# chungimungi/GMLM

Measured on AMD Instinct MI355X. Metric: nodes/sec fwd+bwd (full-batch GraphTextLM step), higher is better.
Workload: dtype bf16; 1 GPU; squirrel-size synthetic graph x1 (N=5201, E=217073, F_in=2089), hidden_channels=768, BERT geometry 768x12, 1257 active text nodes, 16..128 tokens, plm_batch_size=4096; global_nodes=5201, parallelism=single GPU, activation_checkpointing=False, plm_gradient_checkpointing=False, world=1, hip_graph=False, gemm_algorithms=library picks from gmlm_amd/tunable/gfx950.csv (TunableOp lookup)

## Files before the change

gmlm_amd/csrc/wgrad_kernels.hip:

```cpp
#include "attn_common.hpp"

namespace gmlm {

namespace wg {
constexpr int BT = 32;
constexpr int TILE = 256;
constexpr int NW = 8;
constexpr int NBUF = 4;
constexpr int IMG = BT * TILE * 2;
constexpr int STAGE = 2 * IMG;
constexpr int LDS = NBUF * STAGE;
constexpr int PIECES = IMG / 1024 / NW;
constexpr int VM_PER_STAGE = 2 * PIECES;
__device__ __forceinline__ int swz(int r) { return 2 * ((r & 3) | (((r >> 3) & 1) << 2)); }
}

struct WgradParams {
  const bf16_t* dy;
  const bf16_t* x;
  float* part;
  int64_t ld_dy, ld_x, n, k;
  int32_t stages, splits, tiles_k, tiles, remap;
};

__device__ __forceinline__ uint32_t wg_src_off(int64_t ld, int w, int lane) {
  const int row = 2 * w + (lane >> 5), slot = lane & 31;
  return 2u * (uint32_t)(row * ld + 8 * (slot ^ wg::swz(row)));
}

__device__ __forceinline__ void wg_dma(const bf16_t* base, uint32_t off, uint32_t lds) {
  const uint32_t dst = __builtin_amdgcn_readfirstlane(lds);
  uint32_t keep;
  asm volatile("s_mov_b32 %0, m0\n\ts_mov_b32 m0, %3\n\ts_nop 0\n\tglobal_load_lds_dwordx4 %1, %2\n\ts_mov_b32 m0, %0"
               : "=&s"(keep) : "v"(off), "s"(base), "s"(dst) : "memory");
}

__global__ __launch_bounds__(wg::NW * 64, 1) void wgrad_bf16_kernel(WgradParams p) {
  using namespace wg;
  extern __shared__ __attribute__((aligned(1024))) unsigned char smem_dyn[];
  const uint32_t lds0 = (uint32_t)(size_t)(__attribute__((address_space(3))) void*)smem_dyn;
  const int tid = threadIdx.x, lane = tid & 63, w = __builtin_amdgcn_readfirstlane(tid >> 6);
  const uint32_t nwg = gridDim.x, id = blockIdx.x;
  uint32_t lid = id;
  if (p.remap) {
    const uint32_t q = nwg >> 3, r = nwg & 7, xcd = id & 7;
    lid = (xcd < r ? xcd * (q + 1) : r * (q + 1) + (xcd - r) * q) + (id >> 3);
  }
  const int slice = (int)(lid / (uint32_t)p.tiles), tile = (int)(lid % (uint32_t)p.tiles);
  const int n0 = (tile / p.tiles_k) * TILE, k0 = (tile % p.tiles_k) * TILE;
  const int st0 = (int)((int64_t)slice * p.stages / p.splits), st1 = (int)((int64_t)(slice + 1) * p.stages / p.splits);
  const int ns = st1 - st0;

  const uint32_t offa = wg_src_off(p.ld_dy, w, lane), offb = wg_src_off(p.ld_x, w, lane);
  const bf16_t* ga = p.dy + (int64_t)st0 * BT * p.ld_dy + n0;
  const bf16_t* gb = p.x + (int64_t)st0 * BT * p.ld_x + k0;
  const int64_t stepa = (int64_t)BT * p.ld_dy, stepb = (int64_t)BT * p.ld_x;
  auto issue = [&](int s) {
    const uint32_t buf = lds0 + (uint32_t)((s % NBUF) * STAGE) + 1024u * (uint32_t)w;
    const bf16_t* a = ga + s * stepa;
    const bf16_t* b = gb + s * stepb;
#pragma unroll
    for (int k = 0; k < PIECES; ++k) {
      wg_dma(a + (int64_t)(16 * k) * p.ld_dy, offa, buf + 1024u * (uint32_t)(NW * k));
      wg_dma(b + (int64_t)(16 * k) * p.ld_x, offb, buf + (uint32_t)IMG + 1024u * (uint32_t)(NW * k));
    }
  };

  const int g = lane >> 4, q = (lane >> 2) & 3, pp = lane & 3;
  const int wr = w >> 2, wc = w & 3;
  const int row = 8 * g + q, sw = swz(row);
  const uint32_t rbase = (uint32_t)(row * (TILE * 2)) + 8u * (uint32_t)(pp & 1);
  uint32_t aoff[8], boff[4];
#pragma unroll
  for (int m = 0; m < 8; ++m) aoff[m] = rbase + 16u * (uint32_t)((((wr * 128 + 16 * m) >> 3) + (pp >> 1)) ^ sw);
#pragma unroll
  for (int j = 0; j < 4; ++j) boff[j] = (uint32_t)IMG + rbase + 16u * (uint32_t)((((wc * 64 + 16 * j) >> 3) + (pp >> 1)) ^ sw);

  typedef __attribute__((ext_vector_type(4))) float f32x4;
  f32x4 acc[8][4];
#pragma unroll
  for (int m = 0; m < 8; ++m)
#pragma unroll
    for (int j = 0; j < 4; ++j) acc[m][j] = f32x4{0.f, 0.f, 0.f, 0.f};

  const int pre = ns < NBUF - 1 ? ns : NBUF - 1;
  for (int s = 0; s < pre; ++s) issue(s);
  int issued = pre;
  for (int s = 0; s < ns; ++s) {
    const int younger = issued - s - 1;
    if (younger >= 2) asm volatile("s_waitcnt vmcnt(8)" ::: "memory");
    else if (younger == 1) asm volatile("s_waitcnt vmcnt(4)" ::: "memory");
    else asm volatile("s_waitcnt vmcnt(0)" ::: "memory");
    static_assert(VM_PER_STAGE == 4 && NBUF == 4, "vmcnt immediates above assume 4 per stage and 2 younger stages");
    __builtin_amdgcn_s_barrier();
    asm volatile("" ::: "memory");
    if (issued < ns) { issue(issued); ++issued; }
    const unsigned char* img = smem_dyn + (s % NBUF) * STAGE;
    bf16x8 a[8], b[4];
#pragma unroll
    for (int j = 0; j < 4; ++j) {
      const bf16x4 lo = __builtin_amdgcn_ds_read_tr16_b64_v4bf16(GMLM_LDS3(bf16x4, img + boff[j]));
      const bf16x4 hi = __builtin_amdgcn_ds_read_tr16_b64_v4bf16(GMLM_LDS3(bf16x4, img + boff[j] + 4 * TILE * 2));
      b[j] = bf16x8{lo[0], lo[1], lo[2], lo[3], hi[0], hi[1], hi[2], hi[3]};
    }
#pragma unroll
    for (int m = 0; m < 8; ++m) {
      const bf16x4 lo = __builtin_amdgcn_ds_read_tr16_b64_v4bf16(GMLM_LDS3(bf16x4, img + aoff[m]));
      const bf16x4 hi = __builtin_amdgcn_ds_read_tr16_b64_v4bf16(GMLM_LDS3(bf16x4, img + aoff[m] + 4 * TILE * 2));
      a[m] = bf16x8{lo[0], lo[1], lo[2], lo[3], hi[0], hi[1], hi[2], hi[3]};
    }
#pragma unroll
    for (int m = 0; m < 8; ++m)
#pragma unroll
      for (int j = 0; j < 4; ++j) acc[m][j] = __builtin_amdgcn_mfma_f32_16x16x32_bf16(a[m], b[j], acc[m][j], 0, 0, 0);
  }

  float* out = p.part + (int64_t)slice * p.n * p.k + (int64_t)(n0 + wr * 128 + 4 * g) * p.k + k0 + wc * 64 + (lane & 15);
#pragma unroll
  for (int m = 0; m < 8; ++m)
#pragma unroll
    for (int j = 0; j < 4; ++j)
#pragma unroll
      for (int r = 0; r < 4; ++r) out[(int64_t)(16 * m + r) * p.k + 16 * j] = acc[m][j][r];
}

__global__ __launch_bounds__(256) void wgrad_combine_kernel(const float* __restrict__ part, int splits, int64_t n, int64_t k,
                                                            const bf16_t* __restrict__ dy, int64_t ld_dy, const bf16_t* __restrict__ x,
                                                            int64_t ld_x, int64_t t_main, int64_t t, float* __restrict__ out,
                                                            int64_t ld_out) {
  const int64_t k4 = k >> 2, i = (int64_t)blockIdx.x * 256 + threadIdx.x;
  if (i >= n * k4) return;
  const int64_t r = i / k4, c = 4 * (i - r * k4);
  typedef __attribute__((ext_vector_type(4))) float f32x4;
  const int64_t nk = n * k;
  const float* src = part + r * k + c;
  f32x4 s = *reinterpret_cast<const f32x4*>(src);
  for (int j = 1; j < splits; ++j) {
    const f32x4 v = *reinterpret_cast<const f32x4*>(src + j * nk);
#pragma unroll
    for (int e = 0; e < 4; ++e) s[e] = __fadd_rn(s[e], v[e]);
  }
  for (int64_t tt = t_main; tt < t; ++tt) {
    const float a = bf16_to_f32(dy[tt * ld_dy + r]);
    const bf16x4 xb = *reinterpret_cast<const bf16x4*>(x + tt * ld_x + c);
#pragma unroll
    for (int e = 0; e < 4; ++e) s[e] = fmaf(a, (float)xb[e], s[e]);
  }
  *reinterpret_cast<f32x4*>(out + r * ld_out + c) = s;
}

}

using namespace gmlm;

namespace {
int wgrad_splits(int64_t t, int64_t n, int64_t k, int splits) {
  const int64_t tiles = (n / wg::TILE) * (k / wg::TILE), stages = t / wg::BT;
  int64_t s = splits > 0 ? splits : 256 / tiles;
  if (s < 1) s = 1;
  if (s > stages) s = stages;
  return (int)s;
}
}

extern "C" size_t gmlm_wgrad_workspace_bytes(int64_t t, int64_t n, int64_t k, int splits) {
  if (t < wg::BT || n <= 0 || k <= 0) return 0;
  return (size_t)wgrad_splits(t, n, k, splits) * (size_t)n * (size_t)k * sizeof(float);
}

extern "C" int gmlm_wgrad_bf16(const void* dy, int64_t ld_dy, const void* x, int64_t ld_x, int64_t t, int64_t n, int64_t k,
                               int splits, float* out, int64_t ld_out, int flags, void* workspace, size_t workspace_bytes,
                               gmlm_stream_t stream) {
  GMLM_REQUIRE(dy && x && out && workspace, "wgrad_bf16: null pointer");
  GMLM_REQUIRE(t >= wg::BT && n > 0 && k > 0, "wgrad_bf16: need t >= %d and n, k > 0 (t=%lld n=%lld k=%lld)", wg::BT, (long long)t,
               (long long)n, (long long)k);
  GMLM_REQUIRE(n % wg::TILE == 0 && k % wg::TILE == 0, "wgrad_bf16: n and k must be multiples of %d (n=%lld k=%lld)", wg::TILE,
               (long long)n, (long long)k);
  GMLM_REQUIRE(ld_dy >= n && ld_x >= k && ld_out >= k, "wgrad_bf16: row stride smaller than the row");
  GMLM_REQUIRE(ld_dy % 8 == 0 && ld_x % 8 == 0 && ld_out % 4 == 0, "wgrad_bf16: row strides must keep rows 16-byte aligned");
  GMLM_REQUIRE(((uintptr_t)dy | (uintptr_t)x | (uintptr_t)out | (uintptr_t)workspace) % 16 == 0,
               "wgrad_bf16: pointers must be 16-byte aligned");
  GMLM_REQUIRE(splits >= 0 && (flags & ~GMLM_WGRAD_NO_REMAP) == 0, "wgrad_bf16: bad splits / flags");
  GMLM_REQUIRE(ld_dy < (1ll << 26) && ld_x < (1ll << 26), "wgrad_bf16: row stride too large");
  const int s = wgrad_splits(t, n, k, splits);
  const size_t need = (size_t)s * (size_t)n * (size_t)k * sizeof(float);
  if (workspace_bytes < need) {
    set_error("wgrad_bf16: workspace of %zu bytes, need %zu", workspace_bytes, need);
    return GMLM_EWORKSPACE;
  }
  const int64_t tiles_k = k / wg::TILE, tiles = (n / wg::TILE) * tiles_k, stages = t / wg::BT;
  GMLM_REQUIRE(tiles * s < (1ll << 31) && stages < (1ll << 31), "wgrad_bf16: problem too large");
  static std::once_flag once;
  static hipError_t attr = hipSuccess;
  std::call_once(once, [] {
    attr = hipFuncSetAttribute(reinterpret_cast<const void*>(&wgrad_bf16_kernel), hipFuncAttributeMaxDynamicSharedMemorySize, wg::LDS);
  });
  GMLM_HIP(attr);
  hipStream_t st = as_stream(stream);
  WgradParams p{(const bf16_t*)dy, (const bf16_t*)x, (float*)workspace, ld_dy, ld_x, n, k, (int32_t)stages, s, (int32_t)tiles_k,
                (int32_t)tiles, (flags & GMLM_WGRAD_NO_REMAP) ? 0 : 1};
  wgrad_bf16_kernel<<<(unsigned)(tiles * s), wg::NW * 64, wg::LDS, st>>>(p);
  GMLM_LAUNCH_CHECK();
  const int64_t items = n * (k / 4);
  wgrad_combine_kernel<<<(unsigned)((items + 255) / 256), 256, 0, st>>>((const float*)workspace, s, n, k, (const bf16_t*)dy, ld_dy,
                                                                      (const bf16_t*)x, ld_x, stages * wg::BT, t, out, ld_out);
  GMLM_LAUNCH_CHECK();
  return GMLM_OK;
}
```

gmlm_amd/ops.py:

```python
from __future__ import annotations

from typing import Optional

import torch

from . import _lib
from ._lib import BF16, F32, check, lib


def _ptr(t: Optional[torch.Tensor]):
    return None if t is None else t.data_ptr()


def _stream():
    return torch.cuda.current_stream().cuda_stream


def _dt(t: torch.Tensor) -> int:
    if t.dtype == torch.float32:
        return F32
    if t.dtype == torch.bfloat16:
        return BF16
    raise TypeError(f"gmlm_amd kernels take float32 or bfloat16 tensors, got {t.dtype}")


def _cuda(*ts):
    for t in ts:
        if t is not None and not t.is_cuda:
            raise _lib.GmlmHipError("gmlm_amd ops run on the GPU only (tensor on %s); there is no CPU path" % t.device)
    dev = next(t for t in ts if t is not None).device
    _lib.require_gfx950(dev.index if dev.index is not None else torch.cuda.current_device())


def _ws(nbytes: int, device) -> torch.Tensor:
    return torch.empty(max(int(nbytes), 16), dtype=torch.uint8, device=device)


def _f32c(t: torch.Tensor) -> torch.Tensor:
    return t.detach().float().contiguous()


class KernelTimer:

    def __init__(self):
        self.records = []

    def span(self, name, **meta):
        return _Span(self, name, meta)

    def summary(self):
        torch.cuda.synchronize()
        out = {}
        for name, e0, e1, meta in self.records:
            d = out.setdefault(name, dict(launches=0, ms=0.0, bytes=0.0, flops=0.0))
            d["launches"] += 1
            d["ms"] += e0.elapsed_time(e1)
            d["bytes"] += meta.get("bytes", 0.0)
            d["flops"] += meta.get("flops", 0.0)
        return out


class _Span:
    def __init__(self, timer, name, meta):
        self.timer, self.name, self.meta = timer, name, meta

    def __enter__(self):
        self.e0 = torch.cuda.Event(enable_timing=True)
        self.e1 = torch.cuda.Event(enable_timing=True)
        self.e0.record()
        return self

    def __exit__(self, *exc):
        self.e1.record()
        self.timer.records.append((self.name, self.e0, self.e1, self.meta))
        return False


class _NoSpan:
    def __enter__(self):
        return self

    def __exit__(self, *exc):
        return False


TIMER: Optional[KernelTimer] = None
_NOSPAN = _NoSpan()


def _span(name, **meta):
    return TIMER.span(name, **meta) if TIMER is not None else _NOSPAN


def spmm_algorithmic_bytes(num_edges, num_segments, out_rows, f, elem, edge_w=False):
    return float(num_edges * (f * elem + 4 + (4 if edge_w else 0)) + (num_segments + 1) * 4 + out_rows * f * elem)


SEED_DEVICE: Optional[torch.Tensor] = None


def _sd():
    return None if SEED_DEVICE is None else SEED_DEVICE.data_ptr()


def draw_seed() -> int:
    return int(torch.randint(0, 2 ** 62, (1,), device="cpu").item())


def degree(index: torch.Tensor, num_nodes: Optional[int] = None, dtype=torch.float32) -> torch.Tensor:
    _cuda(index)
    index = index.to(torch.long).contiguous()
    if num_nodes is None:
        num_nodes = int(index.max().item()) + 1 if index.numel() else 0
    if dtype == torch.float32:
        out = torch.empty(num_nodes, dtype=torch.float32, device=index.device)
        check(lib().gmlm_degree_f32(_ptr(index), index.numel(), num_nodes, _ptr(out), _stream()), "gmlm_degree_f32")
        return out
    out = torch.empty(num_nodes, dtype=torch.int32, device=index.device)
    check(lib().gmlm_degree_i32(_ptr(index), index.numel(), num_nodes, _ptr(out), _stream()), "gmlm_degree_i32")
    return out.to(dtype)


def edge_types_from_degree(edge_index: torch.Tensor, num_nodes: int) -> torch.Tensor:
    _cuda(edge_index)
    src = edge_index[0].to(torch.long).contiguous()
    e = src.numel()
    deg = torch.empty(num_nodes, dtype=torch.int32, device=src.device)
    check(lib().gmlm_degree_i32(_ptr(src), e, num_nodes, _ptr(deg), _stream()), "gmlm_degree_i32")
    et = torch.empty(e, dtype=torch.long, device=src.device)
    check(lib().gmlm_edge_bucket(_ptr(src), _ptr(deg), e, num_nodes, _ptr(et), _stream()), "gmlm_edge_bucket")
    return et


def _spmm(src, rowptr, idx, edge_w, mean, num_segments, f, out, split=None):
    if split is not None and split.n_long > 0:
        partial = torch.empty(split.n_chunks, f, dtype=torch.float32, device=src.device)
        extra = (split.thresh, _ptr(split.long_seg), _ptr(split.chunk_ptr), _ptr(split.chunk_owner), split.n_long,
                 split.n_chunks, _ptr(partial))
    else:
        extra = (0, None, None, None, 0, 0, None)
    check(lib().gmlm_rgcn_mean_spmm(_ptr(src), src.shape[0], src.stride(0), _ptr(rowptr), _ptr(idx), _ptr(edge_w),
                                    1 if mean else 0, num_segments, f, _ptr(out), f, _dt(src), *extra, _stream()),
          "gmlm_rgcn_mean_spmm")


def column_sum(x: torch.Tensor) -> torch.Tensor:
    _cuda(x)
    x = x.contiguous()
    n, f = x.shape
    out = torch.empty(2, f, dtype=torch.float32, device=x.device)
    if n == 0:
        return out[0].zero_()
    ws = _ws(lib().gmlm_colstats_workspace_bytes(n, f), x.device)
    check(lib().gmlm_colstats(_ptr(x), _dt(x), None, n, f, _ptr(out[0]), _ptr(out[1]), _ptr(ws), ws.numel(), _stream()), "gmlm_colstats")
    return out[0]


WGRAD_TILE = 256
WGRAD_NO_REMAP = 1


def wgrad_bf16(dy: torch.Tensor, x: torch.Tensor, splits: int = 0, flags: int = 0) -> torch.Tensor:
    _cuda(dy, x)
    t, n = dy.shape
    k = x.shape[1]
    out = torch.empty(n, k, dtype=torch.float32, device=dy.device)
    ws = _ws(lib().gmlm_wgrad_workspace_bytes(t, n, k, splits), dy.device)
    check(lib().gmlm_wgrad_bf16(_ptr(dy), dy.stride(0), _ptr(x), x.stride(0), t, n, k, splits, _ptr(out), k, flags, _ptr(ws),
                                ws.numel(), _stream()), "gmlm_wgrad_bf16")
    return out


def device_split_plan(rowptr: torch.Tensor, num_items: int, thresh: int = 64):
    import ctypes
    from .graph import SplitPlan
    cl, cc = ctypes.c_int64(), ctypes.c_int64()
    check(lib().gmlm_split_plan_capacity(int(num_items), int(thresh), ctypes.byref(cl), ctypes.byref(cc)), "gmlm_split_plan_capacity")
    dev = rowptr.device
    long_seg = torch.empty(cl.value, dtype=torch.int32, device=dev)
    chunk_ptr = torch.empty(cl.value + 1, dtype=torch.int32, device=dev)
    chunk_owner = torch.empty(cc.value, dtype=torch.int32, device=dev)
    check(lib().gmlm_split_plan_build(_ptr(rowptr), rowptr.numel() - 1, int(num_items), int(thresh), _ptr(long_seg), _ptr(chunk_ptr),
                                      _ptr(chunk_owner), _stream()), "gmlm_split_plan_build")
    return SplitPlan(int(thresh), long_seg, chunk_ptr, chunk_owner, int(cl.value), int(cc.value))


class RGCNAggregate(torch.autograd.Function):

    @staticmethod
    def forward(ctx, x: torch.Tensor, csr) -> torch.Tensor:
        _cuda(x)
        x = x.contiguous()
        n_src, f = x.shape
        n = csr.num_nodes
        if n_src != csr.num_src:
            raise ValueError(f"x has {n_src} rows but the graph expects {csr.num_src} source rows")
        out = torch.empty(n, csr.r_active * f, dtype=x.dtype, device=x.device)
        with _span("spmm_fwd", bytes=spmm_algorithmic_bytes(csr.num_edges, n * csr.r_active, n * csr.r_active, f,
                                                           x.element_size()), f=f):
            _spmm(x, csr.rowptr, csr.col, None, True, n * csr.r_active, f, out, csr.split)
        ctx.csr, ctx.n_src = csr, x.shape[0]
        return out

    @staticmethod
    def backward(ctx, gh: torch.Tensor):
        csr = ctx.csr
        gh = gh.contiguous()
        n, rf = gh.shape
        f = rf // csr.r_active
        gx = torch.empty(csr.num_src, f, dtype=gh.dtype, device=gh.device)
        with _span("spmm_bwd", bytes=spmm_algorithmic_bytes(csr.num_edges, csr.num_src, csr.num_src, f, gh.element_size(),
                                                           True), f=f):
            _spmm(gh.view(n * csr.r_active, f), csr.t_rowptr, csr.t_seg, csr.inv_cnt, False, csr.num_src, f, gx, csr.t_split)
        return gx, None


GN_ONE_PASS_MAX_RATIO = 64.0


class GraphNormAct(torch.autograd.Function):

    @staticmethod
    def forward(ctx, z, weight, bias, mean_scale, eps, act, p, seed, out_dtype, reducer, n_total):
        _cuda(z)
        z = z.to(out_dtype).contiguous()
        n, f = z.shape
        n_total = int(n_total) if n_total else n
        dev = z.device
        w, b, ms = _f32c(weight), _f32c(bias), _f32c(mean_scale)
        st = _stream()
        dt = _dt(z)
        stats = torch.empty(2, f, dtype=torch.float32, device=dev)
        shift = None
        if reducer is None and n > 0:
            shift = z[0].float().contiguous()
        ws = _ws(lib().gmlm_colstats_workspace_bytes(n, f), dev)
        check(lib().gmlm_colstats(_ptr(z), dt, _ptr(shift), n, f, _ptr(stats[0]), _ptr(stats[1]), _ptr(ws), ws.numel(), st),
              "gmlm_colstats")
        if reducer is not None:
            reducer(stats)
            mu = stats[0] / n_total
            shift = (mu * ms).contiguous()
            check(lib().gmlm_colstats(_ptr(z), dt, _ptr(shift), n, f, _ptr(stats[0]), _ptr(stats[1]), _ptr(ws), ws.numel(),
                                      st), "gmlm_colstats")
            reducer(stats)
            mean = mu.contiguous()
            rstd = torch.rsqrt(stats[1] / n_total + eps).contiguous()
        else:
            mr = torch.empty(2, f, dtype=torch.float32, device=dev)
            check(lib().gmlm_graphnorm_finalize(_ptr(stats[0]), _ptr(stats[1]), _ptr(shift), _ptr(ms), n_total, f, eps,
                                                _ptr(mr[0]), _ptr(mr[1]), st), "gmlm_graphnorm_finalize")
            stats2 = torch.empty_like(stats)
            check(lib().gmlm_colstats(_ptr(z), dt, _ptr(mr[0]), n, f, _ptr(stats2[0]), _ptr(stats2[1]), _ptr(ws), ws.numel(),
                                      st), "gmlm_colstats")
            mr2 = torch.empty_like(mr)
            check(lib().gmlm_graphnorm_finalize(_ptr(stats2[0]), _ptr(stats2[1]), _ptr(mr[0]), _ptr(ms), n_total, f, eps,
                                                _ptr(mr2[0]), _ptr(mr2[1]), st), "gmlm_graphnorm_finalize")
            mr = torch.where(stats[1] * mr[1] * mr[1] > GN_ONE_PASS_MAX_RATIO * n_total, mr2, mr)
            mean, rstd = mr[0], mr[1]
        y = torch.empty(n, f, dtype=out_dtype, device=dev)
        sd = ctx.sd = _sd()
        check(lib().gmlm_graphnorm_apply(_ptr(z), _ptr(mean), _ptr(rstd), _ptr(w), _ptr(b), _ptr(ms), n, f, int(act),
                                         float(p), seed, sd, _ptr(y), dt, st), "gmlm_graphnorm_apply")
        ctx.save_for_backward(z, mean, rstd, w, b, ms)
        ctx.cfg = (int(act), float(p), seed, reducer, n_total)
        return y

    @staticmethod
    def backward(ctx, gy):
        z, mean, rstd, w, b, ms = ctx.saved_tensors
        act, p, seed, reducer, n_total = ctx.cfg
        gy = gy.contiguous().to(z.dtype)
        n, f = z.shape
        dev = z.device
        st = _stream()
        dt = _dt(z)
        gs = torch.empty(2, f, dtype=torch.float32, device=dev)
        ws = _ws(lib().gmlm_colstats_workspace_bytes(n, f), dev)
        sd = ctx.sd
        check(lib().gmlm_graphnorm_bwd_stats(_ptr(gy), dt, _ptr(z), _ptr(mean), _ptr(rstd), _ptr(w), _ptr(b), _ptr(ms),
                                             n, f, act, p, seed, sd, _ptr(gs), _ptr(ws), ws.numel(), st),
              "gmlm_graphnorm_bwd_stats")
        gs_local = gs
        if reducer is not None:
            gs_local = gs.clone()
            reducer(gs)
        dz = torch.empty(n, f, dtype=z.dtype, device=dev)
        if reducer is None:
            dw = torch.empty(f, dtype=torch.float32, device=dev)
            db = torch.empty_like(dw)
            dms = torch.empty_like(dw)
            check(lib().gmlm_graphnorm_bwd_apply(_ptr(gy), dt, _ptr(z), _ptr(mean), _ptr(rstd), _ptr(w), _ptr(b),
                                                 _ptr(ms), _ptr(gs), n, n_total, f, act, p, seed, sd, _ptr(dz), _ptr(dw),
                                                 _ptr(db), _ptr(dms), st), "gmlm_graphnorm_bwd_apply")
        else:
            check(lib().gmlm_graphnorm_bwd_apply(_ptr(gy), dt, _ptr(z), _ptr(mean), _ptr(rstd), _ptr(w), _ptr(b),
                                                 _ptr(ms), _ptr(gs), n, n_total, f, act, p, seed, sd, _ptr(dz), None, None,
                                                 None, st), "gmlm_graphnorm_bwd_apply")
            dw, db = gs_local[1].clone(), gs_local[0].clone()
            m2 = gs[1] / n_total
            sum_oh_local = (z.float().sum(0) - n * mean * ms) * rstd
            dms = -mean * (w * rstd * (gs_local[0] - m2 * sum_oh_local))
        return dz, dw, db, dms, None, None, None, None, None, None, None


class BiasResLayerNorm(torch.autograd.Function):
    @staticmethod
    def forward(ctx, x, bias, residual, gamma, beta, eps, act, p, seed):
        _cuda(x)
        shape = x.shape
        f = shape[-1]
        x2 = x.contiguous().view(-1, f)
        rows = x2.shape[0]
        res2 = None if residual is None else residual.to(x.dtype).contiguous().view(-1, f)
        bf = None if bias is None else _f32c(bias)
        g, b = _f32c(gamma), _f32c(beta)
        y = torch.empty_like(x2)
        mean = torch.empty(rows, dtype=torch.float32, device=x.device)
        rstd = torch.empty_like(mean)
        sd = ctx.sd = _sd()
        check(lib().gmlm_bias_res_layernorm_fwd(_ptr(x2), _ptr(bf), _ptr(res2), _ptr(g), _ptr(b), rows, f, float(eps),
                                                int(act), float(p), seed, sd, _ptr(y), _ptr(mean), _ptr(rstd), _dt(x2), _stream()),
              "gmlm_bias_res_layernorm_fwd")
        ctx.save_for_backward(x2, res2, bf, g, b, mean, rstd)
        ctx.cfg = (int(act), float(p), seed, shape, bias is not None, residual is not None)
        return y.view(shape)

    @staticmethod
    def backward(ctx, gy):
        x2, res2, bf, g, b, mean, rstd = ctx.saved_tensors
        act, p, seed, shape, has_bias, has_res = ctx.cfg
        rows, f = x2.shape
        gy2 = gy.contiguous().view(rows, f).to(x2.dtype)
        dx = torch.empty_like(x2)
        dres = torch.empty_like(x2) if has_res else None
        dg = torch.empty(f, dtype=torch.float32, device=x2.device)
        dbeta = torch.empty_like(dg)
        dbias = torch.empty_like(dg) if has_bias else None
        ws = _ws(lib().gmlm_layernorm_bwd_workspace_bytes(rows, f), x2.device)
        sd = ctx.sd
        check(lib().gmlm_bias_res_layernorm_bwd(_ptr(gy2), _ptr(x2), _ptr(bf), _ptr(res2), _ptr(g), _ptr(b), _ptr(mean),
                                                _ptr(rstd), rows, f, act, p, seed, sd, _ptr(dx), _ptr(dres), _ptr(dg),
                                                _ptr(dbeta), _ptr(dbias), _dt(x2), _ptr(ws), ws.numel(), _stream()),
              "gmlm_bias_res_layernorm_bwd")
        return (dx.view(shape), dbias, None if dres is None else dres.view(shape), dg, dbeta, None, None, None, None)


def bias_res_layernorm(x, bias, residual, gamma, beta, eps=1e-5, act=False, p=0.0, training=False):
    p = float(p) if training else 0.0
    return BiasResLayerNorm.apply(x, bias, residual, gamma, beta, eps, act, p, draw_seed() if p > 0 else 0)


def _rows_view(t: torch.Tensor, h: int, d: int):
    if t.stride(-1) != 1 or t.shape[-1] != h * d:
        raise ValueError("attention operands must be [b, l, h*d] with a contiguous last dim")
    if t.stride(0) != t.shape[1] * t.stride(1) and t.shape[0] > 1:
        raise ValueError("attention operands must have batch stride = l * row stride")
    return t.stride(1)


def _short_path(dtype, d: int, rows: int, pairs: int) -> bool:
    return dtype == torch.bfloat16 and d == 64 and rows <= 128 and pairs >= 512


class Attention(torch.autograd.Function):

    @staticmethod
    def forward(ctx, q, k, v, kv_len, h, scale, p, seed):
        _cuda(q, k, v)
        b, lq, hd = q.shape
        lk = k.shape[1]
        d = hd // h
        qs, ks, vs = _rows_view(q, h, d), _rows_view(k, h, d), _rows_view(v, h, d)
        out = torch.empty(b, lq, hd, dtype=q.dtype, device=q.device)
        lse = torch.empty(b, h, lq, dtype=torch.float32, device=q.device)
        want_lo = q.dtype == torch.bfloat16 and not _short_path(q.dtype, d, max(lq, lk), b * h) and \
            any(t.requires_grad for t in (q, k, v))
        out_lo = torch.empty_like(out) if want_lo else None
        with _span("attn_fwd_d%d" % d, flops=4.0 * b * h * lq * lk * d):
            sd = ctx.sd = _sd()
            if d == 128:
                check(lib().gmlm_attention_d128_fwd(_ptr(q), _ptr(k), _ptr(v), _ptr(kv_len), b, h, lq, lk, d, qs, ks, vs, float(scale),
                                                    float(p), seed, sd, _ptr(out), _ptr(out_lo), _ptr(lse), _dt(q), _stream()),
                      "gmlm_attention_d128_fwd")
            else:
                check(lib().gmlm_attention_fwd(_ptr(q), _ptr(k), _ptr(v), _ptr(kv_len), b, h, lq, lk, d, qs, ks, vs, float(scale),
                                               float(p), seed, sd, _ptr(out), _ptr(out_lo), _ptr(lse), _dt(q), None, 0, None, 0,
                                               _stream()),
                      "gmlm_attention_fwd")
        ctx.save_for_backward(q, k, v, out, lse, kv_len, out_lo)
        ctx.cfg = (h, float(scale), float(p), seed)
        return out

    @staticmethod
    def backward(ctx, gout):
        q, k, v, out, lse, kv_len, out_lo = ctx.saved_tensors
        h, scale, p, seed = ctx.cfg
        b, lq, hd = q.shape
        lk = k.shape[1]
        d = hd // h
        gout = gout.contiguous().to(q.dtype)
        dq = torch.empty(b, lq, hd, dtype=q.dtype, device=q.device)
        dk = torch.empty(b, lk, hd, dtype=q.dtype, device=q.device)
        dv = torch.empty(b, lk, hd, dtype=q.dtype, device=q.device)
        ws = _ws(lib().gmlm_attention_d128_workspace_bytes(b, h, lq) if d == 128 else
                 lib().gmlm_attention_bwd_workspace_bytes(b, h, lq, lk, d), q.device)
        with _span("attn_bwd_d%d" % d, flops=10.0 * b * h * lq * lk * d):
            sd = ctx.sd
            if d == 128:
                check(lib().gmlm_attention_d128_bwd(_ptr(q), _ptr(k), _ptr(v), _ptr(out), _ptr(out_lo), _ptr(gout), _ptr(lse),
                                                    _ptr(kv_len), b, h, lq, lk, d, q.stride(1), k.stride(1), v.stride(1), scale, p,
                                                    seed, sd, _ptr(dq), _ptr(dk), _ptr(dv), hd, hd, hd, _dt(q), _ptr(ws), ws.numel(),
                                                    _stream()),
                      "gmlm_attention_d128_bwd")
            else:
                check(lib().gmlm_attention_bwd(_ptr(q), _ptr(k), _ptr(v), _ptr(out), _ptr(gout), _ptr(lse), _ptr(kv_len), b, h,
                                               lq, lk, d, q.stride(1), k.stride(1), v.stride(1), scale, p, seed, sd, _ptr(dq),
                                               _ptr(dk), _ptr(dv), hd, hd, hd, _dt(q), None, 0, _ptr(ws), ws.numel(), None, None,
                                               _ptr(out_lo), None, 0, _stream()),
                      "gmlm_attention_bwd")
        return dq, dk, dv, None, None, None, None, None


class AttentionQKV(torch.autograd.Function):

    @staticmethod
    def forward(ctx, qkv, kv_len, h, scale, p, seed, cu_seqlens, max_len, pair_count=None, groups=None, *bias_masters):
        _cuda(qkv)
        qkv = qkv.contiguous()
        packed = cu_seqlens is not None
        if packed:
            l, hd3 = qkv.shape
            b = cu_seqlens.numel() - 1
        else:
            b, l, hd3 = qkv.shape
        hd = hd3 // 3
        d = hd // h
        q, k, v = qkv[..., :hd], qkv[..., hd:2 * hd], qkv[..., 2 * hd:]
        out = torch.empty(qkv.shape[:-1] + (hd,), dtype=qkv.dtype, device=qkv.device)
        lse = torch.empty((h, l) if packed else (b, h, l), dtype=torch.float32, device=qkv.device)
        flops = 4.0 * h * d * ((float(pair_count) if pair_count else float(max_len) * l) if packed else float(b) * l * l)
        rows = int(max_len) if packed else l
        short = _short_path(qkv.dtype, d, rows, b * h)
        if groups is not None and not (packed and short):
            groups = None
        n_groups = 0 if groups is None else groups.numel() - 1
        out_lo = torch.empty_like(out) if (qkv.dtype == torch.bfloat16 and not short and qkv.requires_grad) else None
        nb = out.numel() * out.element_size()
        with _span("attn_fwd_d%d" % d, flops=flops, bytes=(4 + (1 if out_lo is not None else 0)) * nb):
            sd = ctx.sd = _sd()
            check(lib().gmlm_attention_fwd(_ptr(q), _ptr(k), _ptr(v), _ptr(kv_len), b, h, l, l, d, hd3, hd3, hd3, float(scale),
                                           float(p), seed, sd, _ptr(out), _ptr(out_lo), _ptr(lse), _dt(qkv), _ptr(cu_seqlens),
                                           int(max_len), _ptr(groups), n_groups, _stream()), "gmlm_attention_fwd")
        if short:
            ctx.save_for_backward(qkv, lse, kv_len, cu_seqlens, groups)
        else:
            ctx.save_for_backward(qkv, lse, kv_len, cu_seqlens, groups, out, out_lo)
        ctx.short = short
        ctx.cfg = (h, float(scale), float(p), seed, int(max_len), b, l, flops)
        ctx.bias_shapes = [(m.shape[0], m.dtype) for m in bias_masters]
        return out

# ... 477 lines not shown
```

include/gmlm_hip.h:

```cpp
#ifndef GMLM_HIP_H
#define GMLM_HIP_H

#include <stddef.h>
#include <stdint.h>

#ifdef __cplusplus
extern "C" {
#endif

#define GMLM_ABI_VERSION 1

enum gmlm_dtype { GMLM_F32 = 0, GMLM_BF16 = 1 };
enum gmlm_status {
  GMLM_OK = 0,
  GMLM_EINVAL = -1,
  GMLM_EWORKSPACE = -2,
  GMLM_ELAUNCH = -3,
  GMLM_EDEVICE = -4
};

typedef void* gmlm_stream_t;

int gmlm_version(void);
const char* gmlm_last_error(void);
int gmlm_device_check(int* cu_count, int* wave_size, char* arch, int arch_len);

int gmlm_degree_i32(const int64_t* index, int64_t e, int64_t n, int32_t* deg, gmlm_stream_t stream);
int gmlm_degree_f32(const int64_t* index, int64_t e, int64_t n, float* deg, gmlm_stream_t stream);
int gmlm_edge_bucket(const int64_t* src, const int32_t* deg, int64_t e, int64_t n, int64_t* edge_type,
                     gmlm_stream_t stream);
int gmlm_relation_histogram(const int64_t* edge_type, int64_t e, int num_relations, int32_t* rel_count,
                            gmlm_stream_t stream);

size_t gmlm_segment_sort_workspace_bytes(int64_t e);
int gmlm_segment_sort(const int64_t* node, const int64_t* rel, const int32_t* rel_remap, int r_active, int64_t e,
                      int64_t num_segments, int32_t* keys, int32_t* perm, int32_t* rowptr, int32_t* bad_flag,
                      void* workspace, size_t workspace_bytes, gmlm_stream_t stream);
int gmlm_gather_i64_to_i32(const int64_t* src, const int32_t* perm, int64_t e, int32_t* out, gmlm_stream_t stream);
int gmlm_gather_i32(const int32_t* src, const int32_t* perm, int64_t e, int32_t* out, gmlm_stream_t stream);
int gmlm_segment_inv_count(const int32_t* rowptr, int64_t num_segments, float* inv_cnt, gmlm_stream_t stream);

int gmlm_split_plan_capacity(int64_t num_items, int64_t long_threshold, int64_t* cap_long, int64_t* cap_chunks);
int gmlm_split_plan_build(const int32_t* rowptr, int64_t num_segments, int64_t num_items, int64_t long_threshold,
                          int32_t* long_seg, int32_t* chunk_ptr, int32_t* chunk_owner, gmlm_stream_t stream);

int gmlm_rgcn_mean_spmm(const void* src, int64_t src_rows, int64_t src_stride, const int32_t* rowptr,
                        const int32_t* idx, const float* edge_w, int mean, int64_t num_segments, int64_t f,
                        void* out, int64_t out_stride, int dtype, int64_t long_threshold, const int32_t* long_seg,
                        const int32_t* chunk_ptr, const int32_t* chunk_owner, int64_t n_long, int64_t n_chunks,
                        float* partial, gmlm_stream_t stream);

int gmlm_basis_compose_fwd(const float* comp, const float* weight, int r_active, int num_bases, int64_t cols,
                           float* w, gmlm_stream_t stream);
size_t gmlm_basis_compose_bwd_workspace_bytes(int r_active, int num_bases, int64_t cols);
int gmlm_basis_compose_bwd(const float* comp, const float* weight, const float* dw, int r_active, int num_bases,
                           int64_t cols, float* dweight, float* dcomp, void* workspace, size_t workspace_bytes,
                           gmlm_stream_t stream);

size_t gmlm_colstats_workspace_bytes(int64_t n, int64_t f);
int gmlm_colstats(const void* x, int dtype, const float* shift, int64_t n, int64_t f, float* s1, float* s2,
                  void* workspace, size_t workspace_bytes, gmlm_stream_t stream);
int gmlm_graphnorm_finalize(const float* s1, const float* s2, const float* shift, const float* mean_scale,
                            int64_t n_total, int64_t f, float eps, float* mean, float* rstd, gmlm_stream_t stream);
int gmlm_graphnorm_apply(const void* x, const float* mean, const float* rstd, const float* weight,
                         const float* bias, const float* mean_scale, int64_t n, int64_t f, int act,
                         float dropout_p, uint64_t seed, const uint64_t* seed_dev, void* y, int dtype, gmlm_stream_t stream);
int gmlm_graphnorm_bwd_stats(const void* g, int dtype, const void* x, const float* mean, const float* rstd,
                             const float* weight, const float* bias, const float* mean_scale, int64_t n, int64_t f,
                             int act, float dropout_p, uint64_t seed, const uint64_t* seed_dev, float* gs ,
                             void* workspace, size_t workspace_bytes, gmlm_stream_t stream);
int gmlm_graphnorm_bwd_apply(const void* g, int dtype, const void* x, const float* mean, const float* rstd,
                             const float* weight, const float* bias, const float* mean_scale, const float* gs,
                             int64_t n, int64_t n_total, int64_t f, int act, float dropout_p, uint64_t seed, const uint64_t* seed_dev,
                             void* dx, float* dweight, float* dbias, float* dmean_scale, gmlm_stream_t stream);

int gmlm_bias_res_layernorm_fwd(const void* x, const float* bias, const void* residual, const float* gamma,
                                const float* beta, int64_t rows, int64_t f, float eps, int act, float dropout_p,
                                uint64_t seed, const uint64_t* seed_dev, void* y, float* mean, float* rstd, int dtype, gmlm_stream_t stream);
size_t gmlm_layernorm_bwd_workspace_bytes(int64_t rows, int64_t f);
int gmlm_bias_res_layernorm_bwd(const void* dy, const void* x, const float* bias, const void* residual,
                                const float* gamma, const float* beta, const float* mean, const float* rstd,
                                int64_t rows, int64_t f, int act, float dropout_p, uint64_t seed, const uint64_t* seed_dev, void* dx,
                                void* dresidual, float* dgamma, float* dbeta, float* dbias, int dtype,
                                void* workspace, size_t workspace_bytes, gmlm_stream_t stream);

int gmlm_attention_fwd(const void* q, const void* k, const void* v, const int32_t* kv_len, int64_t b, int64_t h,
                       int64_t lq, int64_t lk, int64_t d, int64_t q_stride, int64_t k_stride, int64_t v_stride,
                       float scale, float dropout_p, uint64_t seed, const uint64_t* seed_dev, void* out, void* out_lo, float* lse,
                       int dtype, const int32_t* cu_seqlens, int64_t max_len, const int32_t* seq_groups, int64_t num_groups,
                       gmlm_stream_t stream);
size_t gmlm_attention_bwd_workspace_bytes(int64_t b, int64_t h, int64_t lq, int64_t lk, int64_t d);
int gmlm_attention_bwd(const void* q, const void* k, const void* v, const void* out, const void* dout,
                       const float* lse, const int32_t* kv_len, int64_t b, int64_t h, int64_t lq, int64_t lk,
                       int64_t d, int64_t q_stride, int64_t k_stride, int64_t v_stride, float scale,
                       float dropout_p, uint64_t seed, const uint64_t* seed_dev, void* dq, void* dk, void* dv, int64_t dq_stride,
                       int64_t dk_stride, int64_t dv_stride, int dtype, const int32_t* cu_seqlens, int64_t max_len,
                       void* workspace, size_t workspace_bytes,
                       float* dbias_partial , float* dbias ,
                       const void* out_lo, const int32_t* seq_groups, int64_t num_groups, gmlm_stream_t stream);

int gmlm_attention_d128_fwd(const void* q, const void* k, const void* v, const int32_t* kv_len, int64_t b, int64_t h,
                            int64_t lq, int64_t lk, int64_t d, int64_t q_stride, int64_t k_stride, int64_t v_stride,
                            float scale, float dropout_p, uint64_t seed, const uint64_t* seed_dev, void* out,
                            void* out_lo, float* lse, int dtype, gmlm_stream_t stream);
size_t gmlm_attention_d128_workspace_bytes(int64_t b, int64_t h, int64_t lq);
int gmlm_attention_d128_bwd(const void* q, const void* k, const void* v, const void* out, const void* out_lo,
                            const void* dout, const float* lse, const int32_t* kv_len, int64_t b, int64_t h,
                            int64_t lq, int64_t lk, int64_t d, int64_t q_stride, int64_t k_stride, int64_t v_stride,
                            float scale, float dropout_p, uint64_t seed, const uint64_t* seed_dev, void* dq, void* dk,
                            void* dv, int64_t dq_stride, int64_t dk_stride, int64_t dv_stride, int dtype,
                            void* workspace, size_t workspace_bytes, gmlm_stream_t stream);

int gmlm_embed_sum_fwd(const float* word, const float* pos, const float* type0, const int64_t* tok, const int64_t* pos_ids,
                       int64_t rows, int64_t p, int64_t vocab, int64_t npos, void* out, int dtype, int32_t* bad_flag,
                       gmlm_stream_t stream);

int gmlm_meanpool_scatter_fwd(const void* hs, const int32_t* len, const int64_t* node_idx, int64_t b, int64_t l,
                              int64_t p, float* out, int dtype, const int32_t* cu_seqlens, gmlm_stream_t stream);
int gmlm_meanpool_scatter_bwd(const float* dout, const int32_t* len, const int64_t* node_idx, int64_t b, int64_t l,
                              int64_t p, void* dhs, int dtype, const int32_t* cu_seqlens, gmlm_stream_t stream);

int gmlm_softmask_blend_fwd(const float* x, const uint8_t* mask, const float* token, float beta, int64_t n,
                            int64_t f, void* out, int64_t out_stride, int dtype, gmlm_stream_t stream);
int gmlm_softmask_blend_bwd(const float* dout, int64_t dout_stride, const uint8_t* mask, float beta, int64_t n,
                            int64_t f, float* dtoken, void* workspace, size_t workspace_bytes, gmlm_stream_t stream);

int gmlm_bias_gelu_fwd(const void* x, const float* bias, int64_t rows, int64_t f, float dropout_p, uint64_t seed, const uint64_t* seed_dev,
                       void* y, int dtype, gmlm_stream_t stream);
size_t gmlm_bias_gelu_bwd_workspace_bytes(int64_t rows, int64_t f, int dtype);
int gmlm_bias_gelu_bwd(const void* dy, const void* x, const float* bias, int64_t rows, int64_t f, float dropout_p,
                       uint64_t seed, const uint64_t* seed_dev, void* dx, float* dbias, int dtype, void* workspace, size_t workspace_bytes,
                       gmlm_stream_t stream);

#define GMLM_WGRAD_NO_REMAP 1
size_t gmlm_wgrad_workspace_bytes(int64_t t, int64_t n, int64_t k, int splits);
int gmlm_wgrad_bf16(const void* dy, int64_t ld_dy, const void* x, int64_t ld_x, int64_t t, int64_t n, int64_t k, int splits,
                    float* out, int64_t ld_out, int flags, void* workspace, size_t workspace_bytes, gmlm_stream_t stream);

int gmlm_add_rmsnorm_fwd(const void* a, const void* b, const float* w, int64_t rows, int64_t f, float eps, void* s, void* y,
                         float* rstd, int dtype, gmlm_stream_t stream);
size_t gmlm_add_rmsnorm_bwd_workspace_bytes(int64_t rows, int64_t f);
int gmlm_add_rmsnorm_bwd(const void* dy, const void* dres, const void* s, const float* w, const float* rstd, int64_t rows,
                         int64_t f, void* ds, float* dw, int dtype, void* workspace, size_t workspace_bytes,
                         gmlm_stream_t stream);
int gmlm_qknorm_rope_fwd(const void* qkv, int64_t qkv_stride, const float* q_weight, const float* k_weight,
                         const float* cos_sin, int64_t max_len, int64_t tokens, int64_t seq_len, int64_t hq, int64_t hkv,
                         int64_t d, float eps, void* out, int64_t out_stride, float* rstd, int dtype, gmlm_stream_t stream);
size_t gmlm_qknorm_rope_bwd_workspace_bytes(int64_t tokens, int64_t hq, int64_t hkv, int dtype);
int gmlm_qknorm_rope_bwd(void* dqkv, int64_t dqkv_stride, const void* qkv, int64_t qkv_stride, const float* q_weight,
                         const float* k_weight, const float* cos_sin, int64_t max_len, const float* rstd, int64_t tokens,
                         int64_t seq_len, int64_t hq, int64_t hkv, int64_t d, float* dq_weight, float* dk_weight, int dtype,
                         void* workspace, size_t workspace_bytes, gmlm_stream_t stream);
int gmlm_swiglu_fwd(const void* gate_up, int64_t rows, int64_t inter, void* y, int dtype, gmlm_stream_t stream);
int gmlm_swiglu_bwd(const void* dy, const void* gate_up, int64_t rows, int64_t inter, void* dgate_up, int dtype,
                    gmlm_stream_t stream);

int gmlm_attention_causal_d128_fwd(const void* q, const void* k, const void* v, const int32_t* kv_len, int64_t b, int64_t hq,
                                   int64_t hkv, int64_t lq, int64_t lk, int64_t d, int64_t q_stride, int64_t k_stride,
                                   int64_t v_stride, float scale, float dropout_p, void* out, void* out_lo, float* lse,
                                   int dtype, gmlm_stream_t stream);
size_t gmlm_attention_causal_d128_workspace_bytes(int64_t b, int64_t hq, int64_t lq);
int gmlm_attention_causal_d128_bwd(const void* q, const void* k, const void* v, const void* out, const void* out_lo,
                                   const void* dout, const float* lse, const int32_t* kv_len, int64_t b, int64_t hq,
                                   int64_t hkv, int64_t lq, int64_t lk, int64_t d, int64_t q_stride, int64_t k_stride,
                                   int64_t v_stride, float scale, float dropout_p, void* dq, void* dk, void* dv,
                                   int64_t dq_stride, int64_t dk_stride, int64_t dv_stride, int dtype, void* workspace,
                                   size_t workspace_bytes, gmlm_stream_t stream);

#ifdef __cplusplus
}
#endif
#endif
```

Before: 73240 nodes/s.

## Add two-phase ping-pong schedule to wgrad GEMM kernel with wave-group staggering

Adds a templated two-phase variant of the wgrad bf16 kernel and makes it the default. The two wave groups are staggered by one barrier so that one group's LDS reads and memory waits overlap the other group's MFMA burst, with sched_barriers fencing the phases. The aim is to hide LDS-read and vmcnt-wait latency behind matrix-core work. It adds an extra workgroup barrier per stage, and a ONE_PHASE flag is kept to fall back to the old schedule.

```diff
diff --git a/gmlm_amd/csrc/wgrad_kernels.hip b/gmlm_amd/csrc/wgrad_kernels.hip
--- a/gmlm_amd/csrc/wgrad_kernels.hip
+++ b/gmlm_amd/csrc/wgrad_kernels.hip
@@ -35,6 +35,7 @@
                : "=&s"(keep) : "v"(off), "s"(base), "s"(dst) : "memory");
 }
 
+template <bool TWO_PHASE>
 __global__ __launch_bounds__(wg::NW * 64, 1) void wgrad_bf16_kernel(WgradParams p) {
   using namespace wg;
   extern __shared__ __attribute__((aligned(1024))) unsigned char smem_dyn[];
@@ -83,20 +84,16 @@
 #pragma unroll
     for (int j = 0; j < 4; ++j) acc[m][j] = f32x4{0.f, 0.f, 0.f, 0.f};
 
-  const int pre = ns < NBUF - 1 ? ns : NBUF - 1;
-  for (int s = 0; s < pre; ++s) issue(s);
-  int issued = pre;
-  for (int s = 0; s < ns; ++s) {
+  auto wait_stage = [&](int s, int issued) {
     const int younger = issued - s - 1;
     if (younger >= 2) asm volatile("s_waitcnt vmcnt(8)" ::: "memory");
     else if (younger == 1) asm volatile("s_waitcnt vmcnt(4)" ::: "memory");
     else asm volatile("s_waitcnt vmcnt(0)" ::: "memory");
     static_assert(VM_PER_STAGE == 4 && NBUF == 4, "vmcnt immediates above assume 4 per stage and 2 younger stages");
-    __builtin_amdgcn_s_barrier();
-    asm volatile("" ::: "memory");
-    if (issued < ns) { issue(issued); ++issued; }
+  };
+  bf16x8 a[8], b[4];
+  auto read_stage = [&](int s) {
     const unsigned char* img = smem_dyn + (s % NBUF) * STAGE;
-    bf16x8 a[8], b[4];
 #pragma unroll
     for (int j = 0; j < 4; ++j) {
       const bf16x4 lo = __builtin_amdgcn_ds_read_tr16_b64_v4bf16(GMLM_LDS3(bf16x4, img + boff[j]));
@@ -109,10 +106,47 @@
       const bf16x4 hi = __builtin_amdgcn_ds_read_tr16_b64_v4bf16(GMLM_LDS3(bf16x4, img + aoff[m] + 4 * TILE * 2));
       a[m] = bf16x8{lo[0], lo[1], lo[2], lo[3], hi[0], hi[1], hi[2], hi[3]};
     }
+  };
+  auto mma_stage = [&] {
 #pragma unroll
     for (int m = 0; m < 8; ++m)
 #pragma unroll
       for (int j = 0; j < 4; ++j) acc[m][j] = __builtin_amdgcn_mfma_f32_16x16x32_bf16(a[m], b[j], acc[m][j], 0, 0, 0);
+  };
+
+  const int pre = ns < NBUF - 1 ? ns : NBUF - 1;
+  for (int s = 0; s < pre; ++s) issue(s);
+  int issued = pre;
+  if constexpr (!TWO_PHASE) {
+    for (int s = 0; s < ns; ++s) {
+      wait_stage(s, issued);
+      __builtin_amdgcn_s_barrier();
+      asm volatile("" ::: "memory");
+      if (issued < ns) { issue(issued); ++issued; }
+      read_stage(s);
+      mma_stage();
+    }
+  } else {
+    const int grp = w >> 2;
+    if (grp == 1) {
+      wait_stage(0, issued);
+      __builtin_amdgcn_s_barrier();
+    }
+    for (int s = 0; s < ns; ++s) {
+      if (grp == 0) wait_stage(s, issued);
+      __builtin_amdgcn_s_barrier();
+      asm volatile("" ::: "memory");
+      if (issued < ns) { issue(issued); ++issued; }
+      read_stage(s);
+      asm volatile("s_waitcnt lgkmcnt(0)" ::: "memory");
+      if (grp == 1 && s + 1 < ns) wait_stage(s + 1, issued);
+      __builtin_amdgcn_sched_barrier(0);
+      __builtin_amdgcn_s_barrier();
+      __builtin_amdgcn_sched_barrier(0);
+      mma_stage();
+      __builtin_amdgcn_sched_barrier(0);
+    }
+    if (grp == 0) __builtin_amdgcn_s_barrier();
   }
 
   float* out = p.part + (int64_t)slice * p.n * p.k + (int64_t)(n0 + wr * 128 + 4 * g) * p.k + k0 + wc * 64 + (lane & 15);
@@ -180,7 +214,7 @@
   GMLM_REQUIRE(ld_dy % 8 == 0 && ld_x % 8 == 0 && ld_out % 4 == 0, "wgrad_bf16: row strides must keep rows 16-byte aligned");
   GMLM_REQUIRE(((uintptr_t)dy | (uintptr_t)x | (uintptr_t)out | (uintptr_t)workspace) % 16 == 0,
                "wgrad_bf16: pointers must be 16-byte aligned");
-  GMLM_REQUIRE(splits >= 0 && (flags & ~GMLM_WGRAD_NO_REMAP) == 0, "wgrad_bf16: bad splits / flags");
+  GMLM_REQUIRE(splits >= 0 && (flags & ~(GMLM_WGRAD_NO_REMAP | GMLM_WGRAD_ONE_PHASE)) == 0, "wgrad_bf16: bad splits / flags");
   GMLM_REQUIRE(ld_dy < (1ll << 26) && ld_x < (1ll << 26), "wgrad_bf16: row stride too large");
   const int s = wgrad_splits(t, n, k, splits);
   const size_t need = (size_t)s * (size_t)n * (size_t)k * sizeof(float);
@@ -193,13 +227,18 @@
   static std::once_flag once;
   static hipError_t attr = hipSuccess;
   std::call_once(once, [] {
-    attr = hipFuncSetAttribute(reinterpret_cast<const void*>(&wgrad_bf16_kernel), hipFuncAttributeMaxDynamicSharedMemorySize, wg::LDS);
+    attr = hipFuncSetAttribute(reinterpret_cast<const void*>(&wgrad_bf16_kernel<false>), hipFuncAttributeMaxDynamicSharedMemorySize,
+                               wg::LDS);
+    if (attr == hipSuccess)
+      attr = hipFuncSetAttribute(reinterpret_cast<const void*>(&wgrad_bf16_kernel<true>), hipFuncAttributeMaxDynamicSharedMemorySize,
+                                 wg::LDS);
   });
   GMLM_HIP(attr);
   hipStream_t st = as_stream(stream);
   WgradParams p{(const bf16_t*)dy, (const bf16_t*)x, (float*)workspace, ld_dy, ld_x, n, k, (int32_t)stages, s, (int32_t)tiles_k,
                 (int32_t)tiles, (flags & GMLM_WGRAD_NO_REMAP) ? 0 : 1};
-  wgrad_bf16_kernel<<<(unsigned)(tiles * s), wg::NW * 64, wg::LDS, st>>>(p);
+  if (flags & GMLM_WGRAD_ONE_PHASE) wgrad_bf16_kernel<false><<<(unsigned)(tiles * s), wg::NW * 64, wg::LDS, st>>>(p);
+  else wgrad_bf16_kernel<true><<<(unsigned)(tiles * s), wg::NW * 64, wg::LDS, st>>>(p);
   GMLM_LAUNCH_CHECK();
   const int64_t items = n * (k / 4);
   wgrad_combine_kernel<<<(unsigned)((items + 255) / 256), 256, 0, st>>>((const float*)workspace, s, n, k, (const bf16_t*)dy, ld_dy,
diff --git a/gmlm_amd/ops.py b/gmlm_amd/ops.py
--- a/gmlm_amd/ops.py
+++ b/gmlm_amd/ops.py
@@ -158,6 +158,7 @@
 
 WGRAD_TILE = 256
 WGRAD_NO_REMAP = 1
+WGRAD_ONE_PHASE = 2
 
 
 def wgrad_bf16(dy: torch.Tensor, x: torch.Tensor, splits: int = 0, flags: int = 0) -> torch.Tensor:
diff --git a/include/gmlm_hip.h b/include/gmlm_hip.h
--- a/include/gmlm_hip.h
+++ b/include/gmlm_hip.h
@@ -133,6 +133,7 @@
                        gmlm_stream_t stream);
 
 #define GMLM_WGRAD_NO_REMAP 1
+#define GMLM_WGRAD_ONE_PHASE 2
 size_t gmlm_wgrad_workspace_bytes(int64_t t, int64_t n, int64_t k, int splits);
 int gmlm_wgrad_bf16(const void* dy, int64_t ld_dy, const void* x, int64_t ld_x, int64_t t, int64_t n, int64_t k, int splits,
                     float* out, int64_t ld_out, int flags, void* workspace, size_t workspace_bytes, gmlm_stream_t stream);
```

Result: faster. 74000 nodes/s, median of 6 (+1.0%).
